# DiltheyLab/HLA-LA

Hardware: AMD Instinct MI355X
Metric: paired reads/sec aligned to PRG graph (higher is better)
Workload: dtype int32

## Files before the change

### hla-la_amd/csrc/batch.h

```cpp
#pragma once
#include "device_common.h"

namespace hlala {

template <template <class> class Ptr> struct DevBatchT {
    int n_pairs, n_reads, n_chains, stride;
    int from_seeds;
    int unpaired;
    Ptr<const int> read_off;
    Ptr<const uint8_t> read_bases;
    Ptr<const uint8_t> read_quals;
    Ptr<const int> chain_off;
    Ptr<const int> read_primary;
    Ptr<const int> chain_read;
    Ptr<const int> chain_contig;
    Ptr<const int> chain_pos;
    Ptr<const int> chain_offset;
    Ptr<const int> chain_as;
    Ptr<const uint8_t> chain_reverse;
    Ptr<const int> cigar_off;
    Ptr<const u32> cigar;
    Ptr<int> seed_status;
    Ptr<int> seed_ncols;
    Ptr<int> seed_begin;
// ... 29 lines not shown
    Ptr<double> pair_mapq;
    Ptr<double> mate_mapq;
    Ptr<uint8_t> strands_valid;
    Ptr<uint8_t> sel_mapq;
    Ptr<u64> counters;
    Ptr<int> work_counter;
    Ptr<int> retry_list;
    Ptr<int> pair_multi;
    Ptr<uint8_t> pair_deferred;
    Ptr<int> chain_order;
    Ptr<int> chain_bucket;
    Ptr<int> order_hist;
    int order_shift, order_nb;
    int long_chunk_nodes, long_max_segs;
    int order_cost;
    Ptr<int> chain_row;
    int n_rows;
    Ptr<int> dp_blk;
    Ptr<int> dp_list;
    int dp_nblk;
    int dp_band;
    int dp_band_risky;
    int dp_jf;
    Ptr<void> dp_items;
    Ptr<int> dbg;
};
typedef DevBatchT<HostP> DevBatch;
typedef DevBatchT<GlobP> DevBatchG;
static_assert(sizeof(DevBatch) == sizeof(DevBatchG), "one layout");
__device__ __forceinline__ const DevBatchG& dev_view(const DevBatch* p) { return *(const DevBatchG*)p; }
enum { DESC_VALUE = 0, DESC_VIEW = 1, DESC_GENERIC = 2 };
template <int FORM, class D> __device__ __forceinline__ decltype(auto) desc_of(const D& byValue, const D* inMemory)
{
    if constexpr (FORM == DESC_VIEW) return dev_view(inMemory);
    else if constexpr (FORM == DESC_GENERIC) return (*inMemory);
    else return (byValue);
}

template <class BT> __device__ __forceinline__ int ordered_chains(const BT& B) { return B.chain_order ? __builtin_amdgcn_readfirstlane(B.order_hist[B.order_nb - 1]) : B.n_chains; }

template <class BT> __device__ __forceinline__ size_t row_base(const BT& B, int c) { return (size_t)(B.chain_row ? B.chain_row[c] : c) * (size_t)B.stride; }

enum { DPL_BAND16 = 0, DPL_BAND32 = 2, DPL_BAND64 = 4, DPL_JF = 6, DPL_GEN = 8, DPL_N = 10 };
__host__ __device__ inline int dpl_of_class(int cls) { return cls == 0 ? DPL_GEN : (cls == 1 ? DPL_JF : (cls == 2 ? DPL_BAND16 : (cls == 3 ? DPL_BAND32 : DPL_BAND64))); }
enum { WC_PAIR_MULTI = 40, WC_PAIR_OVER = 72, WC_BAND_FETCH = 48, WC_FO_COUNT = 54, WC_FO_FETCH = 56, WC_BAND_FAILED = 58, WC_BAND_CALLS = 59, WC_JF_FAILED = 60, WC_BAND_WHY = 62, WC_BAND_TIED = 68,
       WC_N = 88 };
constexpr int BAND_MAXJ16 = 15, BAND_MAXJ32 = 31, BAND_MAXJ64 = 48;

enum {
    CNT_CHAINS_EXT = 0, CNT_DP_CALLS, CNT_DP_ITERS, CNT_DP_CELLS, CNT_SEED_COLS, CNT_OUT_COLS, CNT_EDGES, CNT_ERRORS, CNT_DP_SHARED
};

}
```

### hla-la_amd/csrc/hlala_api.hip

```cpp
#include <cmath>
#include <cstdio>
#include <cstring>
#include <cstdlib>
#include <algorithm>
#include <map>
#include <mutex>
#include <chrono>
#include <thread>
#include <set>
#include <string>
#include <unordered_map>
#include <vector>

#include "../../include/hlala_gpu.h"
#include "batch.h"
#include "flat_graph.hpp"
#include "host_internal.h"

#include "kernel_dp.hip"
#include "kernel_project.hip"
#include "kernel_order.hip"
#include "kernel_pair.hip"
#include "kernel_pair_overflow.hip"
#include "kernel_typer.hip"
// ... 27 lines not shown

struct hlala_ctx {
    int device = 0;
    hipStream_t stream = nullptr;
    hipStream_t side = nullptr;
    hipStream_t up = nullptr, rs = nullptr, active = nullptr;
    int tail_pool_k = 1; std::vector<hlala_batch*> tail;
    hipEvent_t evSideTail = nullptr; bool sideTailValid = false;
    hlala_params params{};
    FlatGraph F;
    DevGraph G{};
    DevGraph* dG = nullptr;
    DevTables* dT = nullptr;
    double* d_islog = nullptr;
    long long* d_contig_off = nullptr; uint8_t* d_contig_seq = nullptr; int* d_contig_level = nullptr;
    int n_contigs = 0; std::vector<long long> contig_off;
    std::vector<void*> allocs;
    std::unordered_map<void*, size_t> block_bytes;
    std::multimap<size_t, void*> pool;
    size_t pool_bytes = 0;
    size_t pool_cap = (size_t)176 << 30;
    std::mutex pool_mu;
    std::set<struct hlala_batch*> batches;
    int jf_margin = 16;
    int stitch_by_row = 1;
    int stitch_draw = 12;
    bool side_after_pair = false;
    bool rows_all = false;
    bool band_risky = false;
    int band_grid = 0, band_margin = 8;
    DpClass dp[DP_LAST_TIER + 1]; DpClass dp_jf;
    int stitch_grid = 0;
    char* proj_slabs = nullptr; size_t proj_slab_bytes = 0; int proj_grid = 0, pair_grid = 0, pair_lean_grid = 0;
    char* rethread_slabs = nullptr; size_t rethread_slab_bytes = 0; int rethread_grid = 0;
    double* pair_scratch = nullptr;
    char* pair_over_slabs = nullptr; long long pair_over_scratch = 0, pair_over_slab_bytes = 0;
    char* proj_long_slabs = nullptr; size_t proj_long_slab_bytes = 0;
    void* create_scratch = nullptr; size_t create_scratch_bytes = 0; bool create_scratch_pinned = false;
    int long_chunk_nodes = 1 << 20, long_max_segs = 1 << 20;
    int order_cost = 0;
    int order_shift = 8, order_nb = 0;
    int* dbg_host = nullptr;
    int* d_cov = nullptr; int n_cov = 0; int* d_gene_first = nullptr; int* d_gene_last = nullptr; int n_genes = 0;
    struct KeptReads { uint8_t* store = nullptr; long long* start = nullptr; int* length = nullptr; int n = 0; };
    std::vector<KeptReads> kept;
    std::string err;
// ... 329 lines not shown
        rc = dev_upload(c, c->allocs, co.data(), co.size(), &c->d_contig_off); if(rc) return fail(rc);
        rc = dev_upload(c, c->allocs, contigs->contig_seq, total, &c->d_contig_seq); if(rc) return fail(rc);
        rc = dev_upload(c, c->allocs, contigs->contig_level, total, &c->d_contig_level); if(rc) return fail(rc);
    }
    rc = build_tables(c); if(rc) return fail(rc);
    rc = dev_upload(c, c->allocs, &c->G, 1, &c->dG); if(rc) return fail(rc);
    hipDeviceProp_t prop;
    if(hipGetDeviceProperties(&prop, device) != hipSuccess) { c->err = "hipGetDeviceProperties failed"; return fail(HLALA_E_DEVICE); }
    int cus = prop.multiProcessorCount > 0 ? prop.multiProcessorCount : 256;
    auto slab_pool = [&](char** out, size_t bytes, const char* what) -> int {
        if(device_malloc_retry(c->device, nullptr, (void**)out, bytes) != hipSuccess) { c->err = std::string("hipMalloc(") + what + ") failed"; return HLALA_E_DEVICE; }
        c->allocs.push_back(*out);
        if(hipMemsetAsync(*out, 0, bytes, c->active) != hipSuccess) { c->err = std::string("hipMemset(") + what + ") failed"; return HLALA_E_DEVICE; }
        return 0;
    };
    c->band_grid = cus * 20;
    if(const char* e = getenv("HLALA_DP_BAND")) { if(atoi(e) == 0) c->band_grid = 0; }
    if(const char* e = getenv("HLALA_DP_BAND_RISKY")) c->band_risky = atoi(e) != 0;
    if(const char* e = getenv("HLALA_ROWS_ALL")) c->rows_all = atoi(e) != 0;
    if(const char* e = getenv("HLALA_SIDE_AFTER_PAIR")) c->side_after_pair = atoi(e) != 0;
    if(const char* e = getenv("HLALA_POOL_CAP_GB")) { const long g = atol(e); if(g >= 0 && g <= 1024) c->pool_cap = (size_t)g << 30; }
    if(const char* e = getenv("HLALA_DP_BAND_MARGIN")) { const int m = atoi(e); if(m >= 0 && m <= 24) c->band_margin = m; }
    if(const char* e = getenv("HLALA_DP_JF_MARGIN")) { const int m = atoi(e); if(m >= 0 && m <= 200) c->jf_margin = m; }
    c->stitch_grid = cus * 20;
    if(const char* e = getenv("HLALA_STITCH_BY_ROW")) c->stitch_by_row = atoi(e) != 0;
    const size_t extBytes = std::max(dp_slab_bytes<DpSmall>(), dp_slab_bytes<DpWide>()), largeBytes = std::max(dp_slab_bytes<DpLarge>(), dp_slab_bytes<DpBroad>());
    DpClass* const dp = c->dp;
    c->dp_jf = dp_class<DpTinyJF, 0>(cus * 4 * DpTinyJF::WAVES, dp_slab_bytes<DpTiny>(), "k_dp<DpTinyJF>");
    dp[0] = dp_class<DpTiny, 0>(cus * 4 * DpTiny::WAVES, dp_slab_bytes<DpTiny>(), "k_dp<DpTiny>");
    dp[1] = dp_class<DpMid, 1>(cus * 16, dp_slab_bytes<DpMid>(), "k_dp<DpMid>");
    dp[2] = dp_class<DpSmall, 2>(cus * 20, extBytes, "k_dp<DpSmall>");
    dp[3] = dp_class<DpWide, 3>(cus * 7, extBytes, "k_dp<DpWide>");
    dp[4] = dp_class<DpBroad, 4>(cus * 3, largeBytes, "k_dp<DpBroad>");
    dp[5] = dp_class<DpLarge, 5>(cus, largeBytes, "k_dp<DpLarge>");
    dp[6] = dp_class<DpHuge, 6>(cus / 4 > 0 ? cus / 4 : 1, dp_inmemory_bytes<DpHuge>(), "k_dp<DpHuge>");
    if((rc = slab_pool(&dp[0].slabs, dp[0].slab_bytes * (size_t)(64 / DpTiny::GW) * (size_t)std::max(dp[0].grid, c->dp_jf.grid), "16-lane DP slabs"))) return fail(rc);
    c->dp_jf.slabs = dp[0].slabs;
    if((rc = slab_pool(&dp[1].slabs, dp[1].slab_bytes * (size_t)(64 / DpMid::GW) * (size_t)dp[1].grid, "32-lane DP slabs"))) return fail(rc);
    if((rc = slab_pool(&dp[2].slabs, extBytes * (size_t)dp[2].grid, "64-lane DP slabs"))) return fail(rc);
    if((rc = slab_pool(&dp[3].slabs, extBytes * (size_t)dp[3].grid, "wide-class DP slabs"))) return fail(rc);
    if((rc = slab_pool(&dp[4].slabs, largeBytes * (size_t)(dp[4].grid + dp[5].grid), "large-class DP slabs"))) return fail(rc);
    dp[5].slabs = dp[4].slabs + largeBytes * (size_t)dp[4].grid;
    if((rc = slab_pool(&dp[6].slabs, dp[6].slab_bytes * (size_t)dp[6].grid, "in-memory DP class"))) return fail(rc);
    c->proj_grid = cus * (c->params.max_columns <= PROJ_CAP_SHORT ? 12 : 8); c->pair_grid = cus * 16; c->pair_lean_grid = cus * 24;
    { int rcp = dev_alloc(c, c->allocs, (size_t)2 * c->pair_grid * PAIR_COMB, &c->pair_scratch, false); if(rcp) return fail(rcp); }
    if(c->params.max_columns > PROJ_CAP) {
// ... 93 lines not shown
static int batch_alloc_outputs(hlala_ctx* c, hlala_batch* b)
{
    DevBatch& B = b->B;
    size_t nc = (size_t)B.n_chains, nr = (size_t)B.n_reads, np = (size_t)B.n_pairs;
    if(!b->prepared) { B.n_rows = B.n_chains; B.chain_row = nullptr; }
    size_t rowsAlloc = (size_t)(B.n_rows > 0 ? B.n_rows : 1);
    if(b->prepared && nc >= 4096) { const size_t gran = nc / 64; rowsAlloc = (rowsAlloc + gran - 1) / gran * gran; if(rowsAlloc > nc) rowsAlloc = nc; }
    const size_t cs = rowsAlloc * (size_t)B.stride;
    int rc = 0;
#define AL(field, n, zero) do { rc = dev_alloc(c, b->allocs, (n), &B.field, zero); if(rc) return rc; } while(0)
    if(!b->prepared) { AL(seed_status, nc, true); AL(seed_ncols, nc, true); }
    AL(seed_begin, nc, true); AL(seed_end, nc, true); AL(seed_removed, nc, true);
    AL(seed_level, cs, false); AL(seed_edge, cs, false); AL(seed_g, cs, false); AL(seed_s, cs, false);
    AL(ext_status, nc, true); AL(ext_ncols, nc, true); AL(ext_begin, nc, true); AL(ext_end, nc, true); AL(ext_ll, nc, true);
    AL(dp_iters, 2 * nc, true); AL(dp_score, 2 * nc, true); AL(dp_ncols, 2 * nc, true); AL(dp_sb, 2 * nc, true); AL(dp_se, 2 * nc, true); AL(dp_err, 2 * nc, true);
    AL(dp_alias_head, 2 * nc, false); AL(dp_alias_next, 2 * nc, false);
    AL(ext_level, cs, false); AL(ext_edge, cs, false); AL(ext_g, cs, false); AL(ext_s, cs, false); AL(ext_fromseed, cs, false);
    AL(ext_firstlast, 4 * nc, true);
    AL(pair_status, np, true); AL(best_chain, nr, true); AL(n_comb, np, true); AL(pair_ll, np, true); AL(pair_mapq, np, true);
    AL(mate_mapq, nr, true); AL(strands_valid, np, true); AL(sel_mapq, nr * (size_t)B.stride, true);
    AL(pair_deferred, np, true); AL(pair_multi, 7 * np, false); AL(counters, 32, true); AL(work_counter, WC_N, true); AL(retry_list, 16 * nc, false);
    { DpItem* it = nullptr; rc = dev_alloc(c, b->allocs, 2 * nc, &it, false); if(rc) return rc; B.dp_items = it; }
    B.dp_nblk = (int)((nc + 255) / 256); if(B.dp_nblk < 1) B.dp_nblk = 1;
    B.dp_jf = c->jf_margin + 1;
    B.dp_band = c->band_grid > 0 ? c->band_margin + 1 : 0;
    B.dp_band_risky = c->band_risky ? 1 : 0;
    AL(dp_blk, (size_t)DPL_N * B.dp_nblk + 1, false); AL(dp_list, 2 * nc, false);
    if(!b->prepared) {
        B.chain_order = nullptr; B.chain_bucket = nullptr; B.order_hist = nullptr; B.order_shift = c->order_shift; B.order_nb = c->order_nb; B.order_cost = c->order_cost; B.long_chunk_nodes = c->long_chunk_nodes; B.long_max_segs = c->long_max_segs;
        if(c->order_nb > 0 && !B.from_seeds && nc > 0) { AL(chain_order, nc, false); AL(chain_bucket, nc, false); AL(order_hist, (size_t)c->order_nb + 1, false); }
    }
    B.dbg = c->dbg_host;
#undef AL
    return 0;
}

static int batch_create_impl(hlala_ctx* c, const hlala_batch_in* in, hlala_batch** out, bool unpaired);
int hlala_batch_create(hlala_ctx* c, const hlala_batch_in* in, hlala_batch** out) { return batch_create_impl(c, in, out, false); }
int hlala_batch_create_unpaired(hlala_ctx* c, const hlala_batch_in* in, hlala_batch** out) { return batch_create_impl(c, in, out, true); }

static int batch_create_impl(hlala_ctx* c, const hlala_batch_in* in, hlala_batch** out, bool unpaired)
{
    DEV_GUARD(c);
    if(!c || !in || !out) return HLALA_E_ARG;
    UploadScope upscope_(c);
    *out = nullptr;
    if(in->n_pairs < 0 || in->n_chains < 0) { c->err = "negative batch sizes"; return HLALA_E_ARG; }
// ... 935 lines not shown
        if(reset && hipMemset(c->d_cov, 0, nl * sizeof(int)) != hipSuccess) { m->err = "hipMemset failed"; return HLALA_E_DEVICE; } }
    DevGuard g0(c0->device);
    if(hipMemcpy(bases_per_level, m->covAcc, nl * sizeof(int), hipMemcpyDeviceToHost) != hipSuccess) { m->err = "coverage: copy to the host failed"; return HLALA_E_DEVICE; }
    return HLALA_OK;
}


int hlala_batch_get_stats(hlala_ctx* c, hlala_batch* b, hlala_batch_stats* out)
{
    DEV_GUARD(c);
    ReaderScope rscope_(c, b); if(rscope_.rc) return rscope_.rc;
    if(!c || !b || !out) return HLALA_E_ARG;
    memset(out, 0, sizeof(*out));
    if(!b->outputs_ready) return HLALA_OK;
    HIP_TRY(c, hipStreamSynchronize(c->active));
    u64 cnt[16];
    HIP_TRY(c, hipMemcpyAsync(cnt, b->B.counters, sizeof(cnt), hipMemcpyDeviceToHost, c->active)); HIP_TRY(c, hipStreamSynchronize(c->active));
    if((b->staged & 1) && !b->B.from_seeds) (void)hipEventElapsedTime(&out->ms_project, b->ev[EV_PROJECT_BEGIN], b->ev[EV_PROJECT_END]);
    if(b->staged & 2) { (void)hipEventElapsedTime(&out->ms_extend, b->ev[EV_EXTEND_BEGIN], b->ev[EV_EXTEND_END]); if(b->B.n_chains > 0) { (void)hipEventElapsedTime(&out->ms_extend_retry, b->ev[EV_DP_CLASS0_END], b->ev[b->side_used ? EV_DP_CLASS2_END : EV_DP_END]); (void)hipEventElapsedTime(&out->ms_dp_main, b->ev[EV_DP_BEGIN], b->ev[EV_DP_CLASS0_END]);
          for(int k = 0; k <= DP_LAST_TIER; k++) (void)hipEventElapsedTime(&out->ms_dp_class[k], b->ev[EV_DP_CLASS_BEGIN + k], b->ev[EV_DP_CLASS_END + k]);
          (void)hipEventElapsedTime(&out->ms_dp_jump_free, b->ev[EV_DP_CLASS_BEGIN], b->ev[EV_DP_JUMP_FREE_END]);
          if(b->band_used) (void)hipEventElapsedTime(&out->ms_dp_band, b->ev[EV_DP_BAND_BEGIN], b->ev[EV_DP_BAND_END]);
          if(b->side_used) (void)hipEventElapsedTime(&out->ms_side, b->ev[EV_SIDE_BEGIN], b->ev[EV_SIDE_END]); } }
    { int wc[WC_N]; HIP_TRY(c, hipMemcpyAsync(wc, b->B.work_counter, sizeof(wc), hipMemcpyDeviceToHost, c->active)); HIP_TRY(c, hipStreamSynchronize(c->active)); out->n_chains_retried = 0; for(int k = 1; k <= 6; k++) out->n_chains_retried += wc[12 + 4 * (k - 1)] + wc[14 + 4 * (k - 1)]; out->n_dp_retried_large = wc[28] + wc[30];
      out->n_dp_band = b->band_used ? wc[WC_BAND_CALLS] : 0; out->n_dp_band_failed = b->band_used ? wc[WC_BAND_FAILED] : 0; out->n_dp_jump_free_failed = wc[WC_JF_FAILED];
      out->n_dp_class[0] = wc[8] + wc[9] - out->n_dp_band + out->n_dp_band_failed; out->n_dp_jump_free = wc[6]; for(int k = 1; k <= 6; k++) out->n_dp_class[k] = wc[12 + 4 * (k - 1)] + wc[14 + 4 * (k - 1)]; }
    if(b->staged & 4) (void)hipEventElapsedTime(&out->ms_pair, b->ev[EV_PAIR_BEGIN], b->ev[EV_PAIR_END]);
    out->n_chains_extended = (int64_t)cnt[CNT_CHAINS_EXT]; out->n_dp_calls = (int64_t)cnt[CNT_DP_CALLS];
    out->n_dp_iterations = (int64_t)cnt[CNT_DP_ITERS]; out->n_dp_cells = (int64_t)cnt[CNT_DP_CELLS];
    out->n_seed_columns = (int64_t)cnt[CNT_SEED_COLS]; out->n_out_columns = (int64_t)cnt[CNT_OUT_COLS];
    out->n_edges_touched = (int64_t)cnt[CNT_EDGES]; out->n_errors = (int64_t)cnt[CNT_ERRORS]; out->n_dp_shared = (int64_t)cnt[CNT_DP_SHARED];
    return HLALA_OK;
}

}

static int typer_tables(hlala_ctx* c, std::vector<void*>& tmp, TyperTables** out)
{
    TyperTables T;
    double insertionP = c->params.long_read_mode ? 0.075 : 0.001, deletionP = insertionP;
    T.ll_ins_actual = log(insertionP) + log(1.0 / 4.0);
    T.ll_deletion = log(deletionP);
    T.ll_match_mismatch = log(1 - insertionP - deletionP);
    for(int q = 0; q < 256; q++) {
        double pCorrect = host_PhredToPCorrect((unsigned char)(q < 33 ? 33 : q));
        if(pCorrect > 0.999) pCorrect = 0.999;
        if(pCorrect == 0) pCorrect = 0.001;
        T.ll_match[q] = log(pCorrect);
        double pIncorrect = (1 - pCorrect) * (1.0 / 3.0);
// ... 119 lines not shown
    ReaderScope rscope_(c, b); if(rscope_.rc) return rscope_.rc;
    if(!c || !b || !out32) return HLALA_E_ARG;
    if(!b->outputs_ready) { memset(out32, 0, 32 * sizeof(u64)); return HLALA_OK; }
    HIP_TRY(c, hipStreamSynchronize(c->active));
    HIP_TRY(c, hipMemcpyAsync(out32, b->B.counters, 32 * sizeof(u64), hipMemcpyDeviceToHost, c->active)); HIP_TRY(c, hipStreamSynchronize(c->active));
    return HLALA_OK;
}

extern "C" int hlala_debug_memory(hlala_ctx* c, hlala_batch* b, unsigned long long* out4)
{
    if(!c || !out4) return HLALA_E_ARG;
    out4[0] = out4[1] = 0;
    if(b) {
        for(void* p : b->allocs) { auto it = c->block_bytes.find(p); if(it != c->block_bytes.end()) out4[0] += it->second; }
        out4[1] = (unsigned long long)(b->prepared ? b->B.n_rows : b->B.n_chains);
    }
    out4[2] = c->pool_bytes; out4[3] = 0;
    for(auto& kv : c->block_bytes) out4[3] += kv.second;
    return HLALA_OK;
}

extern "C" int hlala_debug_work_counters(hlala_ctx* c, hlala_batch* b, int* out, int capacity)
{
    static_assert(WC_N == HLALA_DEBUG_WC_N && WC_BAND_FETCH == HLALA_DEBUG_WC_BAND_FETCH && WC_BAND_WHY == HLALA_DEBUG_WC_BAND_WHY && WC_BAND_TIED == HLALA_DEBUG_WC_BAND_TIED, "include/hlala_gpu.h: debug section");
    DEV_GUARD(c);
    ReaderScope rscope_(c, b); if(rscope_.rc) return rscope_.rc;
    if(!c || !b || !out || capacity < 0) return HLALA_E_ARG;
    const int n = capacity < WC_N ? capacity : WC_N;
    if(!b->outputs_ready) { memset(out, 0, (size_t)n * sizeof(int)); return HLALA_OK; }
    HIP_TRY(c, hipStreamSynchronize(c->active));
    HIP_TRY(c, hipMemcpyAsync(out, b->B.work_counter, (size_t)n * sizeof(int), hipMemcpyDeviceToHost, c->active)); HIP_TRY(c, hipStreamSynchronize(c->active));
    return HLALA_OK;
}

extern "C" int hlala_debug_dp_items(hlala_ctx* c, hlala_batch* b, int* items_out, long long items_capacity_bytes, int* retry_out, long long retry_capacity_bytes)
{
    DEV_GUARD(c);
    ReaderScope rscope_(c, b); if(rscope_.rc) return rscope_.rc;
    if(!c || !b) return HLALA_E_ARG;
    if(!b->outputs_ready || !(b->staged & 2)) { c->err = "hlala_debug_dp_items before the extension stage"; return HLALA_E_STATE; }
    const size_t nc = (size_t)b->B.n_chains;
    if((items_out && items_capacity_bytes < (long long)(2 * nc * 32)) || (retry_out && retry_capacity_bytes < (long long)(16 * nc * sizeof(int)))) {
        c->err = "hlala_debug_dp_items: buffer too small (items 64 bytes per chain, retry lists 64 bytes per chain)"; return HLALA_E_ARG; }
    if(items_out) HIP_TRY(c, hipMemcpyAsync(items_out, b->B.dp_items, 2 * nc * 32, hipMemcpyDeviceToHost, c->active));
    if(retry_out) HIP_TRY(c, hipMemcpyAsync(retry_out, b->B.retry_list, 16 * nc * sizeof(int), hipMemcpyDeviceToHost, c->active));
    HIP_TRY(c, hipStreamSynchronize(c->active));
    return HLALA_OK;
}

extern "C" int hlala_kat_phred(hlala_ctx* c, int n, const double* p_correct, uint8_t* phred_out, const uint8_t* phred_in, double* p_out)
{
// ... 984 lines not shown
```

### hla-la_amd/csrc/kernel_dp.hip

```cpp
#include "batch.h"
#include "../../include/hlala_gpu.h"

namespace hlala {

enum { K_DIAG = 0, K_GGAP = 1, K_SGAP = 2, K_HOP = 3, K_JUMP = 4 };
enum { M_D = 0, M_GG = 1, M_SG = 2 };
enum { PH_IDLE = 0, PH_RUN, PH_SELECT, PH_BT, PH_EXPAND, PH_DONE };

constexpr u64 HKEY_EMPTY = ~0ull;
#ifndef HLALA_DP_PROFILE_LOG2
#define HLALA_DP_PROFILE_LOG2 18
#endif
#ifndef HLALA_EARLY_GEN_MAX
#define HLALA_EARLY_GEN_MAX 0xFFFFFE
#endif
constexpr int DP_EARLY_GEN_MAX = HLALA_EARLY_GEN_MAX;
constexpr int EXT_PENDING = 0x7FFFFFFF;
constexpr int DP_BT_STEPS_PER_TRIP = 32;

#ifndef HLALA_DP_TAIL_THREADS
#define HLALA_DP_TAIL_THREADS 128
#endif
constexpr int DP_TAIL_THREADS = HLALA_DP_TAIL_THREADS;
#ifndef HLALA_DP_TINY_WAVES
// ... 1310 lines not shown
            }
        }
    }
    bool jfL = false, jfR = false;
    if(needL && B.dp_jf) { const int reach = itL.start_seq + B.dp_jf - 1; jfL = reach < 255 && (int)G.jfree_in[itL.startLevel] > reach; }
    if(needR && B.dp_jf) { const int reach = itR.seqLen - itR.start_seq + B.dp_jf - 1; jfR = reach < 255 && (int)G.jfree_out[itR.startLevel] > reach; }
    bool bdL = false, bdR = false;
    int runL = 0, runR = 0;
    int clsL = jfL ? 1 : 0, clsR = jfR ? 1 : 0;
    if(needL && B.dp_band) { const int jm = itL.start_seq, reach = jm + B.dp_band - 1; runL = (int)G.lin_in[itL.startLevel]; bdL = jm <= BAND_MAXJ64 && runL >= (B.dp_band_risky ? jm : reach + min(jm + 6, 40)); if(bdL) clsL = jm <= BAND_MAXJ16 ? 2 : (jm <= BAND_MAXJ32 ? 3 : 4); }
    if(needR && B.dp_band) { const int jm = itR.seqLen - itR.start_seq, reach = jm + B.dp_band - 1; runR = (int)G.lin_out[itR.startLevel]; bdR = jm <= BAND_MAXJ64 && runR >= (B.dp_band_risky ? jm : reach + min(jm + 6, 40)); if(bdR) clsR = jm <= BAND_MAXJ16 ? 2 : (jm <= BAND_MAXJ32 ? 3 : 4); }
    if(t < nOrd) {
        int4* sl = (int4*)(items + t); int4* sr = (int4*)(items + (size_t)B.n_chains + t);
        if(needL) { sl[0] = make_int4(itL.item, itL.rOff, itL.seqLen, itL.start_seq); sl[1] = make_int4(itL.startLevel, itL.startNode, clsL, runL); } else sl[0] = make_int4(-1, 0, 0, 0);
        if(needR) { sr[0] = make_int4(itR.item, itR.rOff, itR.seqLen, itR.start_seq); sr[1] = make_int4(itR.startLevel, itR.startNode, clsR, runR); } else sr[0] = make_int4(-1, 0, 0, 0);
    }
    __shared__ int blkCnt[DPL_N];
    if(threadIdx.x < DPL_N) blkCnt[threadIdx.x] = 0;
    __syncthreads();
    const int lane = lane_id();
    nShared = wave_sum_i32(nShared);
    if(lane == 0 && nShared) atomicAdd(&B.counters[CNT_DP_SHARED], (u64)nShared);
    const u64 mL = __ballot(needL), mR = __ballot(needR);
    const int kL = needL ? dpl_of_class(clsL) : -1, kR = needR ? dpl_of_class(clsR) + 1 : -1;
    const u64 mJL = __ballot(needL && clsL == 1), mJR = __ballot(needR && clsR == 1), mBL = __ballot(needL && clsL >= 2), mBR = __ballot(needR && clsR >= 2);
    if(lane == 0) {
        if(mL) atomicAdd(&B.work_counter[8], __popcll(mL));
        if(mR) atomicAdd(&B.work_counter[9], __popcll(mR));
        if(mJL | mJR) atomicAdd(&B.work_counter[6], __popcll(mJL) + __popcll(mJR));
        if(mBL | mBR) atomicAdd(&B.work_counter[WC_BAND_CALLS], __popcll(mBL) + __popcll(mBR));
    }
#pragma unroll
    for(int k = 0; k < DPL_N; k++) {
        const u64 mk = __ballot((k & 1) ? kR == k : kL == k);
        if(lane == 0 && mk) atomicAdd(&blkCnt[k], __popcll(mk));
    }
    __syncthreads();
    if(threadIdx.x < DPL_N) B.dp_blk[(size_t)threadIdx.x * gridDim.x + blockIdx.x] = blkCnt[threadIdx.x];
}

__global__ void k_dp_lists(const DevBatch B, const DpItem* __restrict__ items)
{
    const int t = blockIdx.x * blockDim.x + threadIdx.x;
    const int nOrd = ordered_chains(B);
    int kL = -1, kR = -1;
    if(t < nOrd) {
        const int4* sl = (const int4*)(items + t); const int4* sr = (const int4*)(items + (size_t)B.n_chains + t);
        if(sl[0].x >= 0) kL = dpl_of_class(sl[1].z);
        if(sr[0].x >= 0) kR = dpl_of_class(sr[1].z) + 1;
    }
    __shared__ int waveCnt[DPL_N][4];
    const int lane = lane_id(), wv = (int)(threadIdx.x >> 6);
    u64 m[DPL_N];
#pragma unroll
    for(int k = 0; k < DPL_N; k++) m[k] = __ballot((k & 1) ? kR == k : kL == k);
    if(lane == 0) {
#pragma unroll
        for(int k = 0; k < DPL_N; k++) waveCnt[k][wv] = (int)__popcll(m[k]);
    }
    __syncthreads();
    const u64 below = (1ull << lane) - 1ull;
#pragma unroll
    for(int k = 0; k < DPL_N; k++) {
        const bool mine = (k & 1) ? kR == k : kL == k;
        if(mine) {
            int before = 0;
            for(int w2 = 0; w2 < wv; w2++) before += waveCnt[k][w2];
            const int pos = B.dp_blk[(size_t)k * gridDim.x + blockIdx.x] + before + (int)__popcll(m[k] & below);
            B.dp_list[pos] = (k & 1) ? B.n_chains + t : t;
        }
    }
}

struct DpPoolArgs {
    int n;
    u32 seed[DP_POOL_MAX];
    const DevBatch* B[DP_POOL_MAX];
    const DpItem* items[DP_POOL_MAX];
    const uint8_t* bases[DP_POOL_MAX];
};

template <class C, int TIER, class DG, class DB>
__device__ __forceinline__ void dp_class_run(const DG& G, const DB& B, const DpItem* __restrict__ items, DpLdsT<C>& S, DpSlabT<C> sl, u64* sortScratch, const u32 rng_seed,
                                             const int4* __restrict__ nrecOut, const int4* __restrict__ nrecIn, const uint8_t* __restrict__ readBases);

template <class C, int TIER> __host__ __device__ constexpr int dp_desc_form() { return ((TIER == 0 && C::JF) || TIER == 3 || TIER == 5) ? DESC_VIEW : DESC_GENERIC; }

template <class C, int TIER>
__global__ __launch_bounds__(C::THREADS, C::WAVES) void k_dp(const DevGraph* __restrict__ Gp, const DevBatch* __restrict__ Bp, const DpItem* __restrict__ items,
                                                        char* slabs, size_t slabBytes, u32 rng_seed,
                                                        const int4* __restrict__ nrecOut, const int4* __restrict__ nrecIn, const uint8_t* __restrict__ readBasesArg, const DpPoolArgs pool)
{
// ... 28 lines not shown
    constexpr int GW = C::GW;
    constexpr int NG = GW >= 64 ? 1 : 64 / GW;
#ifndef HLALA_DP_DRAW0
#define HLALA_DP_DRAW0 8
#endif
    constexpr int DRAW = (TIER == 0 && C::JF) ? HLALA_DP_DRAW0 : 1;
    const int gl = grp_lane<GW>();

    if(gl == 0) { S.accCalls = 0; S.accIters = 0; S.accCells = 0; S.accEdges = 0; }
#ifdef HLALA_DP_TIMING
    if(gl == 0) { for(int i = 0; i < 16; i++) S.tPh[i] = 0; }
#endif
#ifdef HLALA_DP_TIMING
    long long tAcc[6] = {0, 0, 0, 0, 0, 0}; long long trips = 0, runGroups = 0; long long tMark = clock64();
#define DP_T(i) do { long long t_ = clock64(); tAcc[i] += t_ - tMark; tMark = t_; } while(0)
#else
#define DP_T(i) do { } while(0)
#endif

    constexpr int NPASS = (TIER == 0 && !C::JF) ? 4 : 2;
    for(int pass = 0; pass < NPASS; pass++) {
        const int dirPass = pass & 1;
        const bool foPass = pass >= 2;
        int* fetchCounter = foPass ? &B.work_counter[WC_FO_FETCH + dirPass]
                          : &B.work_counter[TIER == 0 ? (C::JF ? 4 + dirPass : (dirPass ? 10 : 1)) : 13 + 4 * (TIER - 1) + 2 * dirPass];
        const int seg = (C::JF ? DPL_JF : DPL_GEN) + dirPass;
        const bool dense = TIER == 0 && !foPass;
        const int segStart = dense ? uni(B.dp_blk[(size_t)seg * B.dp_nblk]) : 0;
        const int nItems = dense ? uni(B.dp_blk[(size_t)(seg + 1) * B.dp_nblk]) - segStart
                         : (foPass ? uni(B.work_counter[WC_FO_COUNT + dirPass]) : uni(B.work_counter[12 + 4 * (TIER > 0 ? TIER - 1 : 0) + 2 * dirPass]));
        const int* srcList = dense ? B.dp_list + segStart
                           : (foPass ? B.retry_list + (size_t)(14 + dirPass) * (size_t)B.n_chains
                           : B.retry_list + (size_t)(2 * (TIER > 0 ? TIER - 1 : 0) + dirPass) * (size_t)B.n_chains);
        const bool fwd = dirPass != 0;
        if constexpr (DRAW > 1) { if(gl == 0) { S.chunkNext = 0; S.chunkEnd = 0; } DSYNC(); }
        int phase = PH_IDLE;
        bool more = true;
        int edgesAcc = 0;

        for(;;) {
            if(phase == PH_RUN) phase = dp_iterate<C>(S, sl, G, fwd ? nrecOut : nrecIn, readBases, fwd, edgesAcc, sortScratch);
            DP_T(5);
            if(phase == PH_SELECT) phase = dp_select<C>(S, sl, G, rng_seed, fwd);
            DP_T(4);
            if(phase == PH_BT) phase = dp_backtrace<C>(S, sl, DP_BT_STEPS_PER_TRIP, fwd);
            DP_T(3);
            if(phase == PH_EXPAND) phase = dp_expand<C>(S, sl, G, B, fwd ? nrecOut : nrecIn, fwd);
            DP_T(2);
            if(phase == PH_DONE) {
                const int edges = grp_sum_i32<GW>(edgesAcc);
                if(gl == 0) {
                    DpState& st = S.st;
                    S.nextPhase = PH_IDLE;
#ifdef HLALA_DP_PROFILE
                    if(B.dbg && TIER == HLALA_DP_PROFILE && !C::JF) {
                        const long long cyc = clock64() - S.pfStart;
                        if(cyc > (1ll << HLALA_DP_PROFILE_LOG2) && (HLALA_DP_PROFILE_LOG2 >= 12 || (((u32)st.item * 2654435761u) >> 24) == 0)) { int q = atomicAdd(&B.dbg[0], 1); if(q < 500) { int* r = B.dbg + 16 + 16 * q; r[0] = st.item; r[1] = st.itersRun; r[2] = (int)st.cellsEvaluated; r[3] = st.nCells;
                            r[4] = S.pfSlow; r[5] = S.pfImp; r[6] = S.pfPre; r[7] = (int)(cyc >> 10); r[8] = S.pfMaxNT;
                            r[9] = (int)(S.pfPh[4] >> 10); r[10] = (int)(S.pfPh[5] >> 10); r[11] = (int)(S.pfPh[0] >> 10); r[12] = (int)(S.pfPh[3] >> 10); r[13] = (int)(S.pfPh[6] >> 10); r[14] = (int)(S.pfPh[1] >> 10); r[15] = (int)(S.pfPh[2] >> 10); } }
                    }
#endif
                    const bool capacity = st.err != 0 && st.err > -1000000;
                    bool handed = false;
                    if constexpr (C::JF && TIER == 0) if(capacity && S.jumpMet) {
                        if(st.isAlias) ((int*)(items + st.itemIdx))[0] = st.item;
                        const int q = atomicAdd(&B.work_counter[WC_FO_COUNT + dirPass], 1); B.retry_list[(size_t)(14 + dirPass) * (size_t)B.n_chains + q] = st.itemIdx;
                        atomicAdd(&B.work_counter[WC_JF_FAILED], 1);
                        handed = true;
                    }
                    if(handed) { }
                    else if(capacity && TIER < DP_LAST_TIER) {
                        int to = TIER + 1; if(st.needTier > to) to = st.needTier; if(to > DP_LAST_TIER) to = DP_LAST_TIER;
                        int* cnt = &B.work_counter[12 + 4 * (to - 1) + 2 * dirPass]; int* lst = B.retry_list + (size_t)(2 * (to - 1) + dirPass) * (size_t)B.n_chains;
                        if(st.isAlias) ((int*)(items + st.itemIdx))[0] = st.item;
                        int q = atomicAdd(cnt, 1); lst[q] = st.itemIdx;
                        if(to >= DP_SIDE_TIER && B.n_pairs > 0 && !B.unpaired) B.pair_deferred[B.chain_read[st.item >> 1] >> 1] = 1;
                    } else {
                        const int item = st.item;
                        B.dp_iters[item] = st.itersRun; B.dp_score[item] = st.have ? st.endScore : INT32_MIN;
                        B.dp_ncols[item] = st.have ? st.nCols : -1; B.dp_sb[item] = st.sb; B.dp_se[item] = st.se; B.dp_err[item] = st.err;
                        S.accCalls++; S.accIters += (u64)st.itersRun; S.accCells += (u64)st.cellsEvaluated; S.accEdges += (u64)edges;
                        int nx = B.dp_alias_head[item]; if(nx < 0) nx = B.dp_alias_next[item];
                        const bool failed = st.err != 0 && st.err > -1000000;
                        while(nx >= 0 && failed) {
                            B.dp_iters[nx] = st.itersRun; B.dp_score[nx] = INT32_MIN; B.dp_ncols[nx] = -1; B.dp_sb[nx] = st.sb; B.dp_se[nx] = st.se; B.dp_err[nx] = st.err;
                            S.accCalls++; S.accIters += (u64)st.itersRun; S.accCells += (u64)st.cellsEvaluated; S.accEdges += (u64)edges;
                            nx = B.dp_alias_next[nx];
                        }
                        if(nx >= 0) {
                            st.item = nx; st.isAlias = 1;
                            st.endSlot = -1; st.endScore = 0; st.nSteps = 0; st.nCols = 0; st.have = 0; st.sb = 0; st.se = -1; st.err = 0;
                            S.nextPhase = PH_SELECT;
                        }
                    }
                }
                DSYNC();
                phase = guni<GW>(S.nextPhase);
            }
            DP_T(1);
            if(phase == PH_IDLE && more) {
                int w = 0;
                if(gl == 0) {
                    if constexpr (DRAW > 1) {
                        int nx = S.chunkNext;
                        if(nx >= S.chunkEnd) { nx = atomicAdd(fetchCounter, DRAW); S.chunkEnd = nx + DRAW; }
                        S.chunkNext = nx + 1; w = nx;
                    } else w = atomicAdd(fetchCounter, 1);
                }
                w = grp_bcast0<GW>(w);
                if(w >= nItems) more = false;
                else {
                    const int idx = guni<GW>(srcList[w]);
                    const int4* ip = (const int4*)(items + idx);
                    int4 a = ip[0], b = ip[1];
                    DpItem it; it.item = a.x; it.rOff = a.y; it.seqLen = a.z; it.start_seq = a.w; it.startLevel = b.x; it.startNode = b.y; it.pad0 = 0; it.pad1 = 0;
                    phase = dp_begin<C>(S, sl, G, it, idx);
                    edgesAcc = 0;
                }
            }
            DP_T(0);
            if(!__ballot(phase != PH_IDLE)) break;
#ifdef HLALA_DP_TIMING
            trips++; runGroups += __popcll(__ballot(phase == PH_RUN)) / GW;
#endif
            DP_T(5);
        }
    }
    if(gl == 0 && S.accCalls) {
        atomicAdd(&B.counters[CNT_DP_CALLS], S.accCalls); atomicAdd(&B.counters[CNT_DP_ITERS], S.accIters);
        atomicAdd(&B.counters[CNT_DP_CELLS], S.accCells); atomicAdd(&B.counters[CNT_EDGES], S.accEdges);
    }
#ifdef HLALA_DP_TIMING
    if(TIER == 0 && (threadIdx.x & 63) == 0) { for(int i = 0; i < 8; i++) atomicAdd(&B.counters[24 + i], (u64)S.tPh[i]); for(int i = 0; i < 8; i++) atomicAdd(&B.counters[16 + i], (u64)S.tPh[8 + i]);
        for(int i = 0; i < 6; i++) atomicAdd(&B.counters[8 + i], (u64)tAcc[i]); atomicAdd(&B.counters[14], (u64)trips); atomicAdd(&B.counters[15], (u64)runGroups); }
#endif
}

template <int PER, class DB>
__device__ __forceinline__ void stitch_rounds(const DB& B, const DevTables& T, const size_t cb, const int rOff, const int total, const int padL, const int nL, const int nSeed,
                                              const int nR, const int newEnd, const int stride, const int lane, double& llOut, int& f0, int& f1, int& l0, int& l1)
{
    const int seedAt = padL + nL, rightAt = seedAt + nSeed, padRAt = rightAt + nR;
    const int srcShift = (stride - nR) - rightAt;
    double carry = 0.0; int baseIdx = 0;
    f0 = -1; f1 = -1; l0 = -1; l1 = -1;
    for(int c0 = 0; c0 < total; c0 += 64 * PER) {
        const int chunk = min(64 * PER, total - c0);
        const int per = (chunk + 63) / 64;
        const int j0 = c0 + lane * per, j1 = min(c0 + chunk, j0 + per);
        int lv[PER], ed[PER]; unsigned char gcv[PER], scv[PER], kind[PER];
#pragma unroll
        for(int k = 0; k < PER; k++) {
            const int j = j0 + k; const bool in = k < per && j < j1;
            lv[k] = -1; ed[k] = -1; gcv[k] = '_'; scv[k] = '_'; kind[k] = 4;
            if(in) {
// ... 166 lines not shown
```

Before: 5.662 million.

## Split DP work lists by remaining read length so long items start first

Jump-free and general DP items are now placed into separate long and short lists by how many read bases remain in the extension direction, with a threshold that defaults to 48. Retry lists for the higher tiers become two-ended: long items fill from the front and short ones from the back, so the fetch loop takes long items before short ones. This is longest-first scheduling, meant to cut the tail where a few long DP jobs finish late while most workgroups sit idle. The cost is more list bookkeeping and counters, plus an extra timing mode.

Result: faster. 5.741 million, median of 6 (+1.4%).

```diff
diff --git a/hla-la_amd/csrc/batch.h b/hla-la_amd/csrc/batch.h
--- a/hla-la_amd/csrc/batch.h
+++ b/hla-la_amd/csrc/batch.h
@@ -75,6 +75,7 @@
     int dp_band;
     int dp_band_risky;
     int dp_jf;
+    int dp_long;
     Ptr<void> dp_items;
     Ptr<int> dbg;
 };
@@ -94,10 +95,20 @@
 
 template <class BT> __device__ __forceinline__ size_t row_base(const BT& B, int c) { return (size_t)(B.chain_row ? B.chain_row[c] : c) * (size_t)B.stride; }
 
-enum { DPL_BAND16 = 0, DPL_BAND32 = 2, DPL_BAND64 = 4, DPL_JF = 6, DPL_GEN = 8, DPL_N = 10 };
-__host__ __device__ inline int dpl_of_class(int cls) { return cls == 0 ? DPL_GEN : (cls == 1 ? DPL_JF : (cls == 2 ? DPL_BAND16 : (cls == 3 ? DPL_BAND32 : DPL_BAND64))); }
+enum { DPL_BAND16 = 0, DPL_BAND32 = 2, DPL_BAND64 = 4, DPL_JF = 6, DPL_GEN = 10, DPL_N = 14 };
+__host__ __device__ inline int dpl_list(int cls, int dir, bool isLong)
+{
+    if(cls >= 2) return (cls == 2 ? DPL_BAND16 : (cls == 3 ? DPL_BAND32 : DPL_BAND64)) + dir;
+    return (cls == 1 ? DPL_JF : DPL_GEN) + 2 * dir + (isLong ? 0 : 1);
+}
+__host__ __device__ inline int dp_bases_left(int dir, int seqLen, int start_seq) { return dir ? seqLen - start_seq : start_seq; }
+__host__ __device__ inline bool dp_is_long(int dpLong, int dir, int seqLen, int start_seq) { return dpLong > 0 && dp_bases_left(dir, seqLen, start_seq) >= dpLong; }
 enum { WC_PAIR_MULTI = 40, WC_PAIR_OVER = 72, WC_BAND_FETCH = 48, WC_FO_COUNT = 54, WC_FO_FETCH = 56, WC_BAND_FAILED = 58, WC_BAND_CALLS = 59, WC_JF_FAILED = 60, WC_BAND_WHY = 62, WC_BAND_TIED = 68,
-       WC_N = 88 };
+       WC_RETRY_LONG = 88, WC_N = 100 };
+__host__ __device__ inline int wc_retry_short(int tier, int dir) { return 12 + 4 * (tier - 1) + 2 * dir; }
+__host__ __device__ inline int wc_retry_fetch(int tier, int dir) { return 13 + 4 * (tier - 1) + 2 * dir; }
+__host__ __device__ inline int wc_retry_long(int tier, int dir) { return WC_RETRY_LONG + 2 * (tier - 1) + dir; }
+__host__ __device__ inline int retry_entry(int w, int nLong, int nChains) { return w < nLong ? w : nChains - 1 - (w - nLong); }
 constexpr int BAND_MAXJ16 = 15, BAND_MAXJ32 = 31, BAND_MAXJ64 = 48;
 
 enum {
diff --git a/hla-la_amd/csrc/hlala_api.hip b/hla-la_amd/csrc/hlala_api.hip
--- a/hla-la_amd/csrc/hlala_api.hip
+++ b/hla-la_amd/csrc/hlala_api.hip
@@ -73,6 +73,7 @@
     size_t pool_cap = (size_t)176 << 30;
     std::mutex pool_mu;
     std::set<struct hlala_batch*> batches;
+    int dp_long_bases = 48;
     int jf_margin = 16;
     int stitch_by_row = 1;
     int stitch_draw = 12;
@@ -448,6 +449,7 @@
     if(const char* e = getenv("HLALA_POOL_CAP_GB")) { const long g = atol(e); if(g >= 0 && g <= 1024) c->pool_cap = (size_t)g << 30; }
     if(const char* e = getenv("HLALA_DP_BAND_MARGIN")) { const int m = atoi(e); if(m >= 0 && m <= 24) c->band_margin = m; }
     if(const char* e = getenv("HLALA_DP_JF_MARGIN")) { const int m = atoi(e); if(m >= 0 && m <= 200) c->jf_margin = m; }
+    if(const char* e = getenv("HLALA_DP_LONG_BASES")) { const int m = atoi(e); if(m >= 0 && m <= 4096) c->dp_long_bases = m; }
     c->stitch_grid = cus * 20;
     if(const char* e = getenv("HLALA_STITCH_BY_ROW")) c->stitch_by_row = atoi(e) != 0;
     const size_t extBytes = std::max(dp_slab_bytes<DpSmall>(), dp_slab_bytes<DpWide>()), largeBytes = std::max(dp_slab_bytes<DpLarge>(), dp_slab_bytes<DpBroad>());
@@ -587,7 +589,7 @@
     AL(pair_deferred, np, true); AL(pair_multi, 7 * np, false); AL(counters, 32, true); AL(work_counter, WC_N, true); AL(retry_list, 16 * nc, false);
     { DpItem* it = nullptr; rc = dev_alloc(c, b->allocs, 2 * nc, &it, false); if(rc) return rc; B.dp_items = it; }
     B.dp_nblk = (int)((nc + 255) / 256); if(B.dp_nblk < 1) B.dp_nblk = 1;
-    B.dp_jf = c->jf_margin + 1;
+    B.dp_jf = c->jf_margin + 1; B.dp_long = c->dp_long_bases;
     B.dp_band = c->band_grid > 0 ? c->band_margin + 1 : 0;
     B.dp_band_risky = c->band_risky ? 1 : 0;
     AL(dp_blk, (size_t)DPL_N * B.dp_nblk + 1, false); AL(dp_list, 2 * nc, false);
@@ -1569,9 +1571,10 @@
           (void)hipEventElapsedTime(&out->ms_dp_jump_free, b->ev[EV_DP_CLASS_BEGIN], b->ev[EV_DP_JUMP_FREE_END]);
           if(b->band_used) (void)hipEventElapsedTime(&out->ms_dp_band, b->ev[EV_DP_BAND_BEGIN], b->ev[EV_DP_BAND_END]);
           if(b->side_used) (void)hipEventElapsedTime(&out->ms_side, b->ev[EV_SIDE_BEGIN], b->ev[EV_SIDE_END]); } }
-    { int wc[WC_N]; HIP_TRY(c, hipMemcpyAsync(wc, b->B.work_counter, sizeof(wc), hipMemcpyDeviceToHost, c->active)); HIP_TRY(c, hipStreamSynchronize(c->active)); out->n_chains_retried = 0; for(int k = 1; k <= 6; k++) out->n_chains_retried += wc[12 + 4 * (k - 1)] + wc[14 + 4 * (k - 1)]; out->n_dp_retried_large = wc[28] + wc[30];
+    { int wc[WC_N]; HIP_TRY(c, hipMemcpyAsync(wc, b->B.work_counter, sizeof(wc), hipMemcpyDeviceToHost, c->active)); HIP_TRY(c, hipStreamSynchronize(c->active)); out->n_chains_retried = 0; for(int k = 1; k <= 6; k++) out->n_dp_class[k] = wc[wc_retry_short(k, 0)] + wc[wc_retry_short(k, 1)] + wc[wc_retry_long(k, 0)] + wc[wc_retry_long(k, 1)];
+      for(int k = 1; k <= 6; k++) out->n_chains_retried += out->n_dp_class[k]; out->n_dp_retried_large = out->n_dp_class[5];
       out->n_dp_band = b->band_used ? wc[WC_BAND_CALLS] : 0; out->n_dp_band_failed = b->band_used ? wc[WC_BAND_FAILED] : 0; out->n_dp_jump_free_failed = wc[WC_JF_FAILED];
-      out->n_dp_class[0] = wc[8] + wc[9] - out->n_dp_band + out->n_dp_band_failed; out->n_dp_jump_free = wc[6]; for(int k = 1; k <= 6; k++) out->n_dp_class[k] = wc[12 + 4 * (k - 1)] + wc[14 + 4 * (k - 1)]; }
+      out->n_dp_class[0] = wc[8] + wc[9] - out->n_dp_band + out->n_dp_band_failed; out->n_dp_jump_free = wc[6]; }
     if(b->staged & 4) (void)hipEventElapsedTime(&out->ms_pair, b->ev[EV_PAIR_BEGIN], b->ev[EV_PAIR_END]);
     out->n_chains_extended = (int64_t)cnt[CNT_CHAINS_EXT]; out->n_dp_calls = (int64_t)cnt[CNT_DP_CALLS];
     out->n_dp_iterations = (int64_t)cnt[CNT_DP_ITERS]; out->n_dp_cells = (int64_t)cnt[CNT_DP_CELLS];
@@ -1737,11 +1740,11 @@
 
 extern "C" int hlala_debug_work_counters(hlala_ctx* c, hlala_batch* b, int* out, int capacity)
 {
-    static_assert(WC_N == HLALA_DEBUG_WC_N && WC_BAND_FETCH == HLALA_DEBUG_WC_BAND_FETCH && WC_BAND_WHY == HLALA_DEBUG_WC_BAND_WHY && WC_BAND_TIED == HLALA_DEBUG_WC_BAND_TIED, "include/hlala_gpu.h: debug section");
+    static_assert(WC_N >= HLALA_DEBUG_WC_N && WC_BAND_FETCH == HLALA_DEBUG_WC_BAND_FETCH && WC_BAND_WHY == HLALA_DEBUG_WC_BAND_WHY && WC_BAND_TIED == HLALA_DEBUG_WC_BAND_TIED, "include/hlala_gpu.h: debug section");
     DEV_GUARD(c);
     ReaderScope rscope_(c, b); if(rscope_.rc) return rscope_.rc;
     if(!c || !b || !out || capacity < 0) return HLALA_E_ARG;
-    const int n = capacity < WC_N ? capacity : WC_N;
+    const int n = capacity < HLALA_DEBUG_WC_N ? capacity : HLALA_DEBUG_WC_N;
     if(!b->outputs_ready) { memset(out, 0, (size_t)n * sizeof(int)); return HLALA_OK; }
     HIP_TRY(c, hipStreamSynchronize(c->active));
     HIP_TRY(c, hipMemcpyAsync(out, b->B.work_counter, (size_t)n * sizeof(int), hipMemcpyDeviceToHost, c->active)); HIP_TRY(c, hipStreamSynchronize(c->active));
diff --git a/hla-la_amd/csrc/kernel_dp.hip b/hla-la_amd/csrc/kernel_dp.hip
--- a/hla-la_amd/csrc/kernel_dp.hip
+++ b/hla-la_amd/csrc/kernel_dp.hip
@@ -1356,7 +1356,7 @@
     nShared = wave_sum_i32(nShared);
     if(lane == 0 && nShared) atomicAdd(&B.counters[CNT_DP_SHARED], (u64)nShared);
     const u64 mL = __ballot(needL), mR = __ballot(needR);
-    const int kL = needL ? dpl_of_class(clsL) : -1, kR = needR ? dpl_of_class(clsR) + 1 : -1;
+    const int kL = needL ? dpl_list(clsL, 0, dp_is_long(B.dp_long, 0, itL.seqLen, itL.start_seq)) : -1, kR = needR ? dpl_list(clsR, 1, dp_is_long(B.dp_long, 1, itR.seqLen, itR.start_seq)) : -1;
     const u64 mJL = __ballot(needL && clsL == 1), mJR = __ballot(needR && clsR == 1), mBL = __ballot(needL && clsL >= 2), mBR = __ballot(needR && clsR >= 2);
     if(lane == 0) {
         if(mL) atomicAdd(&B.work_counter[8], __popcll(mL));
@@ -1366,7 +1366,7 @@
     }
 #pragma unroll
     for(int k = 0; k < DPL_N; k++) {
-        const u64 mk = __ballot((k & 1) ? kR == k : kL == k);
+        const u64 mk = __ballot(kL == k || kR == k);
         if(lane == 0 && mk) atomicAdd(&blkCnt[k], __popcll(mk));
     }
     __syncthreads();
@@ -1380,14 +1380,15 @@
     int kL = -1, kR = -1;
     if(t < nOrd) {
         const int4* sl = (const int4*)(items + t); const int4* sr = (const int4*)(items + (size_t)B.n_chains + t);
-        if(sl[0].x >= 0) kL = dpl_of_class(sl[1].z);
-        if(sr[0].x >= 0) kR = dpl_of_class(sr[1].z) + 1;
+        const int4 a = sl[0], b = sr[0];
+        if(a.x >= 0) kL = dpl_list(sl[1].z, 0, dp_is_long(B.dp_long, 0, a.z, a.w));
+        if(b.x >= 0) kR = dpl_list(sr[1].z, 1, dp_is_long(B.dp_long, 1, b.z, b.w));
     }
     __shared__ int waveCnt[DPL_N][4];
     const int lane = lane_id(), wv = (int)(threadIdx.x >> 6);
     u64 m[DPL_N];
 #pragma unroll
-    for(int k = 0; k < DPL_N; k++) m[k] = __ballot((k & 1) ? kR == k : kL == k);
+    for(int k = 0; k < DPL_N; k++) m[k] = __ballot(kL == k || kR == k);
     if(lane == 0) {
 #pragma unroll
         for(int k = 0; k < DPL_N; k++) waveCnt[k][wv] = (int)__popcll(m[k]);
@@ -1396,12 +1397,11 @@
     const u64 below = (1ull << lane) - 1ull;
 #pragma unroll
     for(int k = 0; k < DPL_N; k++) {
-        const bool mine = (k & 1) ? kR == k : kL == k;
-        if(mine) {
+        if(kL == k || kR == k) {
             int before = 0;
             for(int w2 = 0; w2 < wv; w2++) before += waveCnt[k][w2];
             const int pos = B.dp_blk[(size_t)k * gridDim.x + blockIdx.x] + before + (int)__popcll(m[k] & below);
-            B.dp_list[pos] = (k & 1) ? B.n_chains + t : t;
+            B.dp_list[pos] = kR == k ? B.n_chains + t : t;
         }
     }
 }
@@ -1476,16 +1476,20 @@
     for(int pass = 0; pass < NPASS; pass++) {
         const int dirPass = pass & 1;
         const bool foPass = pass >= 2;
+        constexpr int RT = TIER > 0 ? TIER : 1;
         int* fetchCounter = foPass ? &B.work_counter[WC_FO_FETCH + dirPass]
-                          : &B.work_counter[TIER == 0 ? (C::JF ? 4 + dirPass : (dirPass ? 10 : 1)) : 13 + 4 * (TIER - 1) + 2 * dirPass];
-        const int seg = (C::JF ? DPL_JF : DPL_GEN) + dirPass;
+                          : &B.work_counter[TIER == 0 ? (C::JF ? 4 + dirPass : (dirPass ? 10 : 1)) : wc_retry_fetch(RT, dirPass)];
+        const int seg = (C::JF ? DPL_JF : DPL_GEN) + 2 * dirPass;
         const bool dense = TIER == 0 && !foPass;
+        const bool twoEnded = TIER > 0;
         const int segStart = dense ? uni(B.dp_blk[(size_t)seg * B.dp_nblk]) : 0;
-        const int nItems = dense ? uni(B.dp_blk[(size_t)(seg + 1) * B.dp_nblk]) - segStart
-                         : (foPass ? uni(B.work_counter[WC_FO_COUNT + dirPass]) : uni(B.work_counter[12 + 4 * (TIER > 0 ? TIER - 1 : 0) + 2 * dirPass]));
+        const int nLong = twoEnded ? uni(B.work_counter[wc_retry_long(RT, dirPass)]) : 0;
+        const int nItems = dense ? uni(B.dp_blk[(size_t)(seg + 2) * B.dp_nblk]) - segStart
+                         : (foPass ? uni(B.work_counter[WC_FO_COUNT + dirPass]) : nLong + uni(B.work_counter[wc_retry_short(RT, dirPass)]));
+        const int nChains = B.n_chains;
         const int* srcList = dense ? B.dp_list + segStart
                            : (foPass ? B.retry_list + (size_t)(14 + dirPass) * (size_t)B.n_chains
-                           : B.retry_list + (size_t)(2 * (TIER > 0 ? TIER - 1 : 0) + dirPass) * (size_t)B.n_chains);
+                           : B.retry_list + (size_t)(2 * (RT - 1) + dirPass) * (size_t)B.n_chains);
         const bool fwd = dirPass != 0;
         if constexpr (DRAW > 1) { if(gl == 0) { S.chunkNext = 0; S.chunkEnd = 0; } DSYNC(); }
         int phase = PH_IDLE;
@@ -1525,9 +1529,10 @@
                     if(handed) { }
                     else if(capacity && TIER < DP_LAST_TIER) {
                         int to = TIER + 1; if(st.needTier > to) to = st.needTier; if(to > DP_LAST_TIER) to = DP_LAST_TIER;
-                        int* cnt = &B.work_counter[12 + 4 * (to - 1) + 2 * dirPass]; int* lst = B.retry_list + (size_t)(2 * (to - 1) + dirPass) * (size_t)B.n_chains;
+                        int* lst = B.retry_list + (size_t)(2 * (to - 1) + dirPass) * (size_t)B.n_chains;
                         if(st.isAlias) ((int*)(items + st.itemIdx))[0] = st.item;
-                        int q = atomicAdd(cnt, 1); lst[q] = st.itemIdx;
+                        if(dp_is_long(B.dp_long, dirPass, st.seqLen, st.start_seq)) { const int q = atomicAdd(&B.work_counter[wc_retry_long(to, dirPass)], 1); lst[q] = st.itemIdx; }
+                        else { const int q = atomicAdd(&B.work_counter[wc_retry_short(to, dirPass)], 1); lst[B.n_chains - 1 - q] = st.itemIdx; }
                         if(to >= DP_SIDE_TIER && B.n_pairs > 0 && !B.unpaired) B.pair_deferred[B.chain_read[st.item >> 1] >> 1] = 1;
                     } else {
                         const int item = st.item;
@@ -1564,7 +1569,7 @@
                 w = grp_bcast0<GW>(w);
                 if(w >= nItems) more = false;
                 else {
-                    const int idx = guni<GW>(srcList[w]);
+                    const int idx = guni<GW>(srcList[twoEnded ? retry_entry(w, nLong, nChains) : w]);
                     const int4* ip = (const int4*)(items + idx);
                     int4 a = ip[0], b = ip[1];
                     DpItem it; it.item = a.x; it.rOff = a.y; it.seqLen = a.z; it.start_seq = a.w; it.startLevel = b.x; it.startNode = b.y; it.pad0 = 0; it.pad1 = 0;
@@ -1584,7 +1589,13 @@
         atomicAdd(&B.counters[CNT_DP_CALLS], S.accCalls); atomicAdd(&B.counters[CNT_DP_ITERS], S.accIters);
         atomicAdd(&B.counters[CNT_DP_CELLS], S.accCells); atomicAdd(&B.counters[CNT_EDGES], S.accEdges);
     }
-#ifdef HLALA_DP_TIMING
+#if defined(HLALA_DP_TIMING) && HLALA_DP_TIMING + 0 == 2
+    if(TIER <= 3 && (threadIdx.x & 63) == 0) {
+        constexpr int KI = TIER == 0 ? (C::JF ? 0 : 1) : TIER + 1;
+        const u64 now = (u64)wall_clock64();
+        atomicMax((unsigned long long*)&B.counters[16 + 2 * KI], (unsigned long long)~now); atomicMax((unsigned long long*)&B.counters[17 + 2 * KI], (unsigned long long)now);
+    }
+#elif defined(HLALA_DP_TIMING)
     if(TIER == 0 && (threadIdx.x & 63) == 0) { for(int i = 0; i < 8; i++) atomicAdd(&B.counters[24 + i], (u64)S.tPh[i]); for(int i = 0; i < 8; i++) atomicAdd(&B.counters[16 + i], (u64)S.tPh[8 + i]);
         for(int i = 0; i < 6; i++) atomicAdd(&B.counters[8 + i], (u64)tAcc[i]); atomicAdd(&B.counters[14], (u64)trips); atomicAdd(&B.counters[15], (u64)runGroups); }
 #endif
```
